# mrluin/TextualDegRemoval

Hardware: AMD Instinct MI355X
Metric: train images/sec (512x512, bs=4/GPU) (higher is better)
Workload: dtype f32 (3xbf16-split MFMA: 24-bit operand significands on the full fp32 exponent range, fp32 accumulate; unscaled gradients, no loss scale, no step-skip guard; tensors fp32 -- the MASA-encoder ResidualBlock activations / gradients as three bf16 planes whose sum IS the fp32 value, bit for bit)

## Files before the change

textualdegremoval_amd/csrc/tdr_wgrad_p16.hip:

```cpp
#include <stdlib.h>
#include <stdint.h>
#include "tdr_common.h"
#include "../../include/tdr.h"

typedef _Float16 wf16x8 __attribute__((ext_vector_type(8)));
typedef __bf16 wbf16x8 __attribute__((ext_vector_type(8)));
typedef short ws16x4 __attribute__((ext_vector_type(4)));
typedef short ws16x8 __attribute__((ext_vector_type(8)));

namespace {

struct WgP16Args {
    const uint4* in; const uint4* dout;
    int Cin, Cout, H, W, Hp, Wp;
    int strips, chunks, rc;
    float* part; float* dbpart;
    const void* grp_tab; int grp_pairs, grp_nsplit, grp_units, tiles_co, tiles_ci;
};

#define WGP_GLDS(gptr, lptr)                                                                          \
    __builtin_amdgcn_global_load_lds((__attribute__((address_space(1))) const void*)(gptr),          \
                                     (__attribute__((address_space(3))) void*)(lptr), 16, 0, 0)

__device__ __forceinline__ ws16x8 tr_frag(const char* p, int off0, int off1) {
    const ws16x4 a = __builtin_amdgcn_ds_read_tr16_b64_v4i16((__attribute__((address_space(3))) ws16x4*)(p + off0));
    const ws16x4 b = __builtin_amdgcn_ds_read_tr16_b64_v4i16((__attribute__((address_space(3))) ws16x4*)(p + off1));
    const ws16x8 v = {a[0], a[1], a[2], a[3], b[0], b[1], b[2], b[3]};
    return v;
}
template <int NS>
__device__ __forceinline__ f32x16 wg_mfma(ws16x8 x, ws16x8 y, f32x16 c) {
    if constexpr (NS == 3) return __builtin_amdgcn_mfma_f32_32x32x16_bf16(__builtin_bit_cast(wbf16x8, x), __builtin_bit_cast(wbf16x8, y), c, 0, 0, 0);
    else return __builtin_amdgcn_mfma_f32_32x32x16_f16(__builtin_bit_cast(wf16x8, x), __builtin_bit_cast(wf16x8, y), c, 0, 0, 0);
}

template <int WM, int WN, int WK, int NS = 2, bool GRP = false>
__global__ __launch_bounds__(256, 2) void wgrad3x3_p16_kernel(WgP16Args a) {
    static_assert(WM * WN * WK == 4, "4 waves");
    constexpr int RS = WK == 4 ? 2 : 1;
    static_assert(2 * RS % WK == 0, "k-steps of a step split evenly over the K waves");
    constexpr int BMo = 32 * WM, BNi = 32 * WN, NOo = BMo / 8, NOi = BNi / 8;
    constexpr int XS = 2 * RS + 2, DS = 2 * RS;
    constexpr int XR = ((NOi * NS * 34 + 63) / 64) * 64;
    constexpr int DR = NOo * NS * 32;
    constexpr int XP = XR / 64, DP = DR / 64;

    extern __shared__ __attribute__((aligned(1024))) uint4 smem4[];
    uint4* sX = smem4;
    uint4* sD = smem4 + XS * XR;

    const int tid = threadIdx.x, lane = tid & 63, wave = __builtin_amdgcn_readfirstlane(tid >> 6);
    const int wk = wave % WK, wn = (wave / WK) % WN, wm = wave / (WK * WN);
    int split = blockIdx.x, u0 = blockIdx.x, u1 = u0 + 1, tco = blockIdx.y, tci = blockIdx.z;
    float* dbout = a.dbpart;
    if constexpr (GRP) {
        const int T = a.tiles_co * a.tiles_ci;
        const int c8 = (int)blockIdx.x / (8 * T), r = (int)blockIdx.x - c8 * (8 * T);
        const int pair = c8 * 8 + (r & 7), tile = r >> 3;
        if (pair >= a.grp_pairs) return;
        const int prob = pair / a.grp_nsplit;
        split = pair - prob * a.grp_nsplit;
        tco = tile % a.tiles_co; tci = tile / a.tiles_co;
        u0 = (int)((long)split * a.grp_units / a.grp_nsplit);
        u1 = (int)((long)(split + 1) * a.grp_units / a.grp_nsplit);
        const TdrWg1GroupEntry e = static_cast<const TdrWg1GroupEntry*>(a.grp_tab)[prob];
        a.in = reinterpret_cast<const uint4*>(e.in); a.dout = reinterpret_cast<const uint4*>(e.dout);
        const bool direct = a.grp_nsplit == 1;
        a.part = direct ? e.g : e.part;
        dbout = direct ? e.db : e.dbpart;
    }
    const int co0 = tco * BMo, ci0 = tci * BNi;
    const long PS = (long)a.Hp * a.Wp;
    const int Gi = a.Cin >> 3, Go = a.Cout >> 3;
    const char* xbase = reinterpret_cast<const char*>(a.in);
    const char* dbase = reinterpret_cast<const char*>(a.dout);

    const int nn = lane & 15, g16 = lane >> 4;
    const int jpx = nn >> 2, q = nn & 3, chalf = g16 & 1, kk = g16 >> 1;
    const int oct = chalf * 2 + (q >> 1);
    const int a_lane = ((wm * 4 + oct) * NS * 32 + 8 * kk + jpx) * 16 + (q & 1) * 8;
    const int b_lane = ((wn * 4 + oct) * NS * 34 + 8 * kk + jpx) * 16 + (q & 1) * 8;

    f32x16 acc[9];
#pragma unroll
    for (int tp = 0; tp < 9; ++tp)
#pragma unroll
        for (int r = 0; r < 16; ++r) acc[tp][r] = 0.f;
    f32x16 accb;
#pragma unroll
    for (int r = 0; r < 16; ++r) accb[r] = 0.f;
    const bool want_db = dbout != nullptr && tci == 0 && wn == 0;
    ws16x8 ones;
#pragma unroll
    for (int e = 0; e < 8; ++e) ones[e] = NS == 3 ? (short)0x3f80 : (short)0x3c00;

    for (int u = u0; u < u1; ++u) {
        const int chunk = u % a.chunks; const int t = u / a.chunks;
        const int strip = t % a.strips;
        const int n = t / a.strips;
        const int y0 = chunk * a.rc, y1 = min(y0 + a.rc, a.H);
        const int x0 = strip * 32;

        constexpr int XPW = (XP + 3) / 4, DPW = (DP + 3) / 4;
        unsigned xoff[XPW], doff[DPW];
        const char* xb = xbase + (long)n * Gi * NS * PS * 16;
        const char* db = dbase + (long)n * Go * NS * PS * 16;
        bool dcol[DPW];
#pragma unroll
        for (int i = 0; i < XPW; ++i) {
            const int f = min((wave + 4 * i) * 64 + lane, NOi * NS * 34 - 1);
            const int op = f / 34, c = f - op * 34;
            const int oc = min((ci0 >> 3) + (op / NS), Gi - 1);
            xoff[i] = (unsigned)((((long)oc * NS + (op % NS)) * PS + min(x0 + c, a.Wp - 1)) * 16);
        }
#pragma unroll
        for (int i = 0; i < DPW; ++i) {
            const int f = (wave + 4 * i) * 64 + lane;
            const int op = f >> 5, c = f & 31;
            const int oc = min((co0 >> 3) + (op / NS), Go - 1);
            dcol[i] = x0 + c < a.W;
            doff[i] = (unsigned)((((long)oc * NS + (op % NS)) * PS) * 16);
        }
        auto glds = [&](const char* base, unsigned off, uint4* dst) {
            const unsigned l = (unsigned)(uintptr_t)(__attribute__((address_space(3))) char*)dst;
            unsigned keep;
            asm volatile("s_mov_b32 %0, m0\n\ts_mov_b32 m0, %2\n\ts_nop 0\n\tglobal_load_lds_dwordx4 %1, %3\n\ts_mov_b32 m0, %0"
                         : "=&s"(keep) : "v"(off), "s"(l), "s"(base) : "memory");
        };
        auto issue_x_row = [&](int prow) {
            uint4* dst = sX + (prow % XS) * XR;
            const long rowb = (long)min(prow, a.Hp - 1) * a.Wp * 16;
#pragma unroll
            for (int i = 0; i < XPW; ++i)
                if (wave + 4 * i < XP) glds(xb + rowb, xoff[i], dst + (wave + 4 * i) * 64);
        };
        auto issue_d_row = [&](int y) {
            uint4* dst = sD + (y % DS) * DR;
            const bool yok = y < a.H;
            const unsigned rowb = (unsigned)(((long)(y + 1) * a.Wp + x0 + 1) * 16);
#pragma unroll
            for (int i = 0; i < DPW; ++i)
                if (wave + 4 * i < DP) {
                    const int c = ((wave + 4 * i) * 64 + lane) & 31;
                    glds(db, doff[i] + ((yok && dcol[i]) ? rowb + c * 16 : 0u), dst + (wave + 4 * i) * 64);
                }
        };

        issue_x_row(y0); issue_x_row(y0 + 1);
#pragma unroll
        for (int r = 0; r < RS; ++r) { issue_x_row(y0 + 2 + r); issue_d_row(y0 + r); }
        asm volatile("s_waitcnt vmcnt(0) lgkmcnt(0)\n\ts_barrier" ::: "memory");

        for (int y = y0; y < y1; y += RS) {
#pragma unroll
            for (int r = 0; r < RS; ++r) { issue_x_row(y + RS + 2 + r); issue_d_row(y + RS + r); }
#pragma unroll
            for (int uu = 0; uu < 2 * RS / WK; ++uu) {
                const int ku = wk + uu * WK;
                const int yr = y + (ku >> 1), ks = ku & 1;
                if (yr < y1) {
                    const char* pd = reinterpret_cast<const char*>(sD + (yr % DS) * DR) + a_lane + ks * 256;
                    ws16x8 ap[NS];
#pragma unroll
                    for (int s = 0; s < NS; ++s) ap[s] = tr_frag(pd, s * 32 * 16, s * 32 * 16 + 64);
                    if (want_db) {
#pragma unroll
                        for (int s = NS - 1; s >= 0; --s) accb = wg_mfma<NS>(ap[s], ones, accb);
                    }
                    constexpr int NPR = NS == 3 ? 6 : 3;
                    constexpr int PA[6] = {NS == 3 ? 2 : 1, 0, NS == 3 ? 1 : 0, 1, 0, 0};
                    constexpr int PB[6] = {0, NS == 3 ? 2 : 1, NS == 3 ? 1 : 0, 0, 1, 0};
#pragma unroll
                    for (int ky = 0; ky < 3; ++ky) {
                        const char* px = reinterpret_cast<const char*>(sX + ((yr + ky) % XS) * XR) + b_lane + ks * 256;
                        ws16x8 bp[NS][3];
#pragma unroll
                        for (int s = 0; s < NS; ++s)
#pragma unroll
                            for (int kx = 0; kx < 3; ++kx) bp[s][kx] = tr_frag(px, s * 34 * 16 + kx * 16, s * 34 * 16 + kx * 16 + 64);
#pragma unroll
                        for (int pr = 0; pr < NPR; ++pr)
#pragma unroll
                            for (int kx = 0; kx < 3; ++kx) acc[ky * 3 + kx] = wg_mfma<NS>(ap[PA[pr]], bp[PB[pr]][kx], acc[ky * 3 + kx]);
                    }
                }
            }
            asm volatile("s_waitcnt vmcnt(0) lgkmcnt(0)\n\ts_barrier" ::: "memory");
        }
    }

    const int j = lane & 31, kg = lane >> 5;
    if constexpr (WK > 1) {
        float* red = reinterpret_cast<float*>(smem4);
#pragma unroll
        for (int w = 1; w < WK; ++w) {
            __syncthreads();
            if (wk == w) {
#pragma unroll
                for (int tp = 0; tp < 9; ++tp)
#pragma unroll
                    for (int r = 0; r < 16; ++r) red[(tp * 16 + r) * 64 + lane] = acc[tp][r];
#pragma unroll
                for (int r = 0; r < 16; ++r) red[(9 * 16 + r) * 64 + lane] = accb[r];
            }
            __syncthreads();
            if (wk == 0) {
#pragma unroll
                for (int tp = 0; tp < 9; ++tp)
#pragma unroll
                    for (int r = 0; r < 16; ++r) acc[tp][r] += red[(tp * 16 + r) * 64 + lane];
#pragma unroll
                for (int r = 0; r < 16; ++r) accb[r] += red[(9 * 16 + r) * 64 + lane];
            }
        }
        if (wk != 0) return;
    }
    float* part = a.part + (long)split * a.Cout * a.Cin * 9;
    const int ci = ci0 + wn * 32 + j;
#pragma unroll
    for (int r = 0; r < 16; ++r) {
        const int co = co0 + wm * 32 + (r & 3) + 8 * (r >> 2) + 4 * kg;
        if (co < a.Cout && ci < a.Cin) {
#pragma unroll
            for (int tp = 0; tp < 9; ++tp) part[((long)co * a.Cin + ci) * 9 + tp] = acc[tp][r];
        }
        if (want_db && j == 0 && co < a.Cout) dbout[(long)split * a.Cout + co] = accb[r];
    }
}

template <int KL>
__device__ __forceinline__ void wgp_reduce_block(const float* __restrict__ part, long elems, int nsplit, float* __restrict__ out, int nb_main,
                                                 const float* __restrict__ part2, long elems2, float* __restrict__ out2, int bx) {
    __shared__ float red[KL][64];
    const int lane = threadIdx.x & 63, kl = threadIdx.x >> 6;
    const bool second = bx >= nb_main;
    const float* pbase = second ? part2 : part;
    const long ne = second ? elems2 : elems;
    float* o = second ? out2 : out;
    const long e = (bx - (second ? nb_main : 0)) * 64L + lane;
    const float* p = pbase + (e < ne ? e : ne - 1);
    float s0 = 0.f;
    for (int k = kl; k < nsplit; k += 8 * KL) {
        float v[8];
#pragma unroll
        for (int u = 0; u < 8; ++u) v[u] = k + u * KL < nsplit ? p[(long)(k + u * KL) * ne] : 0.f;
        s0 += ((v[0] + v[1]) + (v[2] + v[3])) + ((v[4] + v[5]) + (v[6] + v[7]));
    }
    red[kl][lane] = s0;
    __syncthreads();
    if (kl == 0 && e < ne) {
        float t = 0.f;
#pragma unroll
        for (int q = 0; q < KL; ++q) t += red[q][lane];
        o[e] = t;
    }
}

template <int KL>
__global__ __launch_bounds__(64 * KL) void wgrad_p16_reduce_kernel(const float* __restrict__ part, long elems, int nsplit, float* __restrict__ out,
                                                                   int nb_main, const float* __restrict__ part2, long elems2, float* __restrict__ out2) {
    wgp_reduce_block<KL>(part, elems, nsplit, out, nb_main, part2, elems2, out2, (int)blockIdx.x);
}

template <int KL>
__global__ __launch_bounds__(64 * KL) void wgrad_p16_reduce_kernel_grp(const TdrWg1GroupEntry* __restrict__ tab, long elems, int nsplit, int Cout,
                                                                       int nb_main) {
    const TdrWg1GroupEntry e = tab[blockIdx.y];
    if ((int)blockIdx.x >= nb_main && (e.db == nullptr || e.dbpart == nullptr)) return;
    wgp_reduce_block<KL>(e.part, elems, nsplit, e.g, nb_main, e.dbpart, (long)Cout, e.db, (int)blockIdx.x);
}

struct WgP16Plan { int cfg, bm, bn, strips, chunks, rc, nsplit; };

long wgp_want_total() {
    static const long want_total = tdr_tune_env("TDR_WGP_WANT") ? atol(tdr_tune_env("TDR_WGP_WANT")) : 512;
    return want_total;
}

WgP16Plan wgp_plan_for(const TdrWgradP16Desc* d, long want) {
    WgP16Plan p;
    p.cfg = (d->Cin <= 32 && d->Cout <= 32) ? 1 : 0;
    p.bm = p.cfg == 1 ? 32 : 64; p.bn = p.bm;
    const int rs = p.cfg == 1 ? 2 : 1;
    p.strips = tdr_cdiv(d->W, 32);
    if (want < 1) want = 1;
    const long rows = (long)d->N * p.strips * d->H;
    long rc = (rows + want - 1) / want;
    if (rc < 8) rc = 8;
    rc = (rc + rs - 1) / rs * rs;
    if (rc > d->H) rc = (d->H + rs - 1) / rs * rs;
    p.rc = (int)rc;
    p.chunks = tdr_cdiv(d->H, p.rc);
    p.nsplit = d->N * p.strips * p.chunks;
    return p;
}

bool wgp_image_fits(const TdrWgradP16Desc* d) {
    const long c = d->Cin > d->Cout ? d->Cin : d->Cout;
    return c / 8 * 3 * (long)(d->H + 2) * (d->W + 2) * 16 < (1L << 32);
}

long wgp_out_tiles(const TdrWgradP16Desc* d) {
    const int t = (d->Cin <= 32 && d->Cout <= 32) ? 32 : 64;
    return (long)tdr_cdiv(d->Cout, t) * tdr_cdiv(d->Cin, t);
}

WgP16Plan wgp_plan(const TdrWgradP16Desc* d) { return wgp_plan_for(d, wgp_want_total() / wgp_out_tiles(d)); }

struct WgP16GroupPlan { WgP16Plan p; int units, nsplit; };

WgP16GroupPlan wgp_group_plan(const TdrWgradP16Desc* d, int nprob) {
    WgP16GroupPlan gp;
    long want = wgp_want_total() / ((long)nprob * wgp_out_tiles(d));
    if (want < 1) want = 1;
    gp.p = wgp_plan_for(d, want);
    gp.units = gp.p.nsplit;
    gp.nsplit = (int)(want < gp.units ? want : gp.units);
    return gp;
}

template <int WM, int WN, int WK, int NS, bool GRP = false>
int launch_wgp(const WgP16Args& a, const WgP16Plan& p, const TdrWgradP16Desc* d, hipStream_t st) {
    constexpr int RS = WK == 4 ? 2 : 1, NOo = 4 * WM, NOi = 4 * WN;
    constexpr int XR = ((NOi * NS * 34 + 63) / 64) * 64, DR = NOo * NS * 32;
    size_t lds = (size_t)((2 * RS + 2) * XR + 2 * RS * DR) * 16;
    if (WK > 1 && lds < 10 * 16 * 64 * 4) lds = 10 * 16 * 64 * 4;
    dim3 grid(p.nsplit, tdr_cdiv(d->Cout, 32 * WM), tdr_cdiv(d->Cin, 32 * WN));
    if (GRP) grid = dim3((unsigned)tdr_cdiv(a.grp_pairs, 8) * 8 * a.tiles_co * a.tiles_ci);
    auto kern = wgrad3x3_p16_kernel<WM, WN, WK, NS, GRP>;
    static bool attr_set = false;
    if (!attr_set) {
        (void)hipFuncSetAttribute(reinterpret_cast<const void*>(kern), hipFuncAttributeMaxDynamicSharedMemorySize, 160 * 1024);
        attr_set = true;
    }
    hipLaunchKernelGGL(kern, grid, dim3(256), lds, st, a);
    TDR_LAUNCH_CHECK(GRP ? "wgrad3x3_p16_kernel<grouped>" : "wgrad3x3_p16_kernel");
    return TDR_OK;
}

}

extern "C" int64_t tdr_wgrad3x3_p16_ws_floats(const TdrWgradP16Desc* d) {
    const WgP16Plan p = wgp_plan(d);
    return (int64_t)p.nsplit * d->Cout * d->Cin * 9 + (int64_t)p.nsplit * d->Cout;
}

extern "C" int tdr_wgrad3x3_p16(const TdrWgradP16Desc* d, void* stream) {
    TDR_REQUIRE(d && d->in16 && d->dout16 && d->g && d->ws, "tdr_wgrad3x3_p16: null pointer");
    TDR_REQUIRE(d->Cin % 16 == 0 && d->Cout % 16 == 0, "tdr_wgrad3x3_p16: channel counts must be multiples of 16 (%d, %d)", d->Cin, d->Cout);
    TDR_REQUIRE(wgp_image_fits(d), "tdr_wgrad3x3_p16: a plane image of more than 4 GiB");
    const WgP16Plan p = wgp_plan(d);
    const int64_t need = tdr_wgrad3x3_p16_ws_floats(d);
    TDR_REQUIRE(d->ws_floats >= need, "tdr_wgrad3x3_p16: workspace too small (%lld < %lld)", (long long)d->ws_floats, (long long)need);
    WgP16Args a;
    a.in = (const uint4*)d->in16; a.dout = (const uint4*)d->dout16;
    a.Cin = d->Cin; a.Cout = d->Cout; a.H = d->H; a.W = d->W; a.Hp = d->H + 2; a.Wp = d->W + 2;
    a.strips = p.strips; a.chunks = p.chunks; a.rc = p.rc;
    a.part = d->ws;
    a.grp_tab = nullptr; a.grp_pairs = a.grp_nsplit = a.grp_units = a.tiles_co = a.tiles_ci = 0;
    a.dbpart = d->db ? d->ws + (int64_t)p.nsplit * d->Cout * d->Cin * 9 : nullptr;
    hipStream_t st = (hipStream_t)stream;
    TDR_REQUIRE(d->fmt == 0 || d->fmt == 1 || d->fmt == 2, "tdr_wgrad3x3_p16: plane format %d (1: bf16 triple, 2: fp16 pair)", d->fmt);
    int rc;
    if (d->fmt == 1) rc = p.cfg == 1 ? launch_wgp<1, 1, 4, 3>(a, p, d, st) : launch_wgp<2, 2, 1, 3>(a, p, d, st);
    else rc = p.cfg == 1 ? launch_wgp<1, 1, 4, 2>(a, p, d, st) : launch_wgp<2, 2, 1, 2>(a, p, d, st);
    if (rc != TDR_OK) return rc;
    const long elems = (long)d->Cout * d->Cin * 9;
    const int nb_main = tdr_cdiv(elems, 64), nb2 = d->db ? tdr_cdiv(d->Cout, 64) : 0;
    if (p.nsplit <= 8)
        hipLaunchKernelGGL(wgrad_p16_reduce_kernel<1>, dim3(nb_main + nb2), dim3(64), 0, st, d->ws, elems, p.nsplit, d->g, nb_main, a.dbpart,
                           (long)d->Cout, d->db);
    else if (p.nsplit <= 64)
        hipLaunchKernelGGL(wgrad_p16_reduce_kernel<4>, dim3(nb_main + nb2), dim3(256), 0, st, d->ws, elems, p.nsplit, d->g, nb_main, a.dbpart,
                           (long)d->Cout, d->db);
    else
        hipLaunchKernelGGL(wgrad_p16_reduce_kernel<16>, dim3(nb_main + nb2), dim3(1024), 0, st, d->ws, elems, p.nsplit, d->g, nb_main, a.dbpart,
                           (long)d->Cout, d->db);
    TDR_LAUNCH_CHECK("wgrad_p16_reduce_kernel");
    return TDR_OK;
}

extern "C" int64_t tdr_wgrad3x3_p16_group_ws_floats(const TdrWgradP16Desc* d, int nprob) {
    if (!d || nprob < 1) return 0;
    const WgP16GroupPlan gp = wgp_group_plan(d, nprob);
    if (gp.nsplit == 1) return 0;
    return (int64_t)gp.nsplit * d->Cout * d->Cin * 9 + (int64_t)gp.nsplit * d->Cout;
}

extern "C" int tdr_wgrad3x3_p16_group_plan(const TdrWgradP16Desc* d, int nprob, int* nsplit, int* units, int* units_per_wg) {
    TDR_REQUIRE(d && nprob > 0, "tdr_wgrad3x3_p16_group_plan: null argument");
    const WgP16GroupPlan gp = wgp_group_plan(d, nprob);
    if (nsplit) *nsplit = gp.nsplit;
    if (units) *units = gp.units;
    if (units_per_wg) *units_per_wg = tdr_cdiv(gp.units, gp.nsplit);
    return TDR_OK;
}

extern "C" int tdr_wgrad3x3_p16_group(const TdrWgradP16Desc* d, int nprob, const void* table, void* stream) {
    TDR_REQUIRE(d && table && nprob > 0, "tdr_wgrad3x3_p16_group: null argument");
    TDR_REQUIRE(d->Cin % 16 == 0 && d->Cout % 16 == 0, "tdr_wgrad3x3_p16_group: channel counts must be multiples of 16 (%d, %d)", d->Cin, d->Cout);
    TDR_REQUIRE(d->fmt == 0 || d->fmt == 1 || d->fmt == 2, "tdr_wgrad3x3_p16_group: plane format %d (1: bf16 triple, 2: fp16 pair)", d->fmt);
    TDR_REQUIRE(wgp_image_fits(d), "tdr_wgrad3x3_p16_group: a plane image of more than 4 GiB");
    const WgP16GroupPlan gp = wgp_group_plan(d, nprob);
    const WgP16Plan& p = gp.p;
    WgP16Args a;
    a.in = nullptr; a.dout = nullptr; a.part = nullptr; a.dbpart = nullptr;
    a.Cin = d->Cin; a.Cout = d->Cout; a.H = d->H; a.W = d->W; a.Hp = d->H + 2; a.Wp = d->W + 2;
    a.strips = p.strips; a.chunks = p.chunks; a.rc = p.rc;
    a.grp_tab = table; a.grp_nsplit = gp.nsplit; a.grp_units = gp.units;
    a.tiles_co = tdr_cdiv(d->Cout, p.bm); a.tiles_ci = tdr_cdiv(d->Cin, p.bn);
    const long pairs = (long)nprob * gp.nsplit;
    TDR_REQUIRE(pairs * a.tiles_co * a.tiles_ci < (1L << 30), "tdr_wgrad3x3_p16_group: too many workgroups (%ld pairs)", pairs);
    a.grp_pairs = (int)pairs;
    hipStream_t st = (hipStream_t)stream;
    int rc;
    if (d->fmt == 1) rc = p.cfg == 1 ? launch_wgp<1, 1, 4, 3, true>(a, p, d, st) : launch_wgp<2, 2, 1, 3, true>(a, p, d, st);
    else rc = p.cfg == 1 ? launch_wgp<1, 1, 4, 2, true>(a, p, d, st) : launch_wgp<2, 2, 1, 2, true>(a, p, d, st);
    if (rc != TDR_OK || gp.nsplit == 1) return rc;
    const long elems = (long)d->Cout * d->Cin * 9;
    const int nb_main = tdr_cdiv(elems, 64), nb2 = tdr_cdiv(d->Cout, 64);
    const TdrWg1GroupEntry* tab = static_cast<const TdrWg1GroupEntry*>(table);
    if (gp.nsplit <= 8)
        hipLaunchKernelGGL(wgrad_p16_reduce_kernel_grp<1>, dim3(nb_main + nb2, nprob), dim3(64), 0, st, tab, elems, gp.nsplit, d->Cout, nb_main);
    else if (gp.nsplit <= 64)
        hipLaunchKernelGGL(wgrad_p16_reduce_kernel_grp<4>, dim3(nb_main + nb2, nprob), dim3(256), 0, st, tab, elems, gp.nsplit, d->Cout, nb_main);
    else
        hipLaunchKernelGGL(wgrad_p16_reduce_kernel_grp<16>, dim3(nb_main + nb2, nprob), dim3(1024), 0, st, tab, elems, gp.nsplit, d->Cout, nb_main);
    TDR_LAUNCH_CHECK("wgrad_p16_reduce_kernel_grp");
    return TDR_OK;
}
```

Before: 62.94.

## Pad and swizzle LDS layout, software-pipeline transposed reads against MFMAs in wgrad

Moves the wgrad LDS geometry into a shared layout header. For the 3-plane case the X-row pitch is padded from 34 to 36, and the dout rows get an XOR rotation by octet to reduce LDS bank conflicts on ds_read_tr. The inner tap loop is rewritten as a statically unrolled, double-buffered pipeline: B fragments for the next tap and A fragments for the next k-step load while the current tap's MFMAs issue. This is steered by sched_group_barrier and stepped s_setprio. It adds register pressure from the double buffers and a static_assert on the LDS budget, and it changes the fill and read addressing that both sides must agree on.

```diff
diff --git a/profiles/wgrad_p16_lds/compare_dumps.py b/profiles/wgrad_p16_lds/compare_dumps.py
--- /dev/null
+++ b/profiles/wgrad_p16_lds/compare_dumps.py
@@ -0,0 +1,17 @@
+import hashlib
+import os
+import sys
+
+import numpy as np
+
+a, b = sys.argv[1:3]
+bad = 0
+print(f'{a} vs {b}')
+for name in ('loss.npy', 'output.npy', 'params.npy'):
+    x, y = np.load(os.path.join(a, name)), np.load(os.path.join(b, name))
+    same = x.shape == y.shape and x.tobytes() == y.tobytes()
+    diff = '' if same else f' max|d|={np.abs(x.astype(np.float64) - y.astype(np.float64)).max():.3e}'
+    print(f'{name} {x.shape} {"IDENTICAL" if same else "DIFFERENT"}{diff} sha256 {hashlib.sha256(x.tobytes()).hexdigest()[:16]} / '
+          f'{hashlib.sha256(y.tobytes()).hexdigest()[:16]}')
+    bad += not same
+sys.exit(1 if bad else 0)
diff --git a/profiles/wgrad_p16_lds/hash_outputs.py b/profiles/wgrad_p16_lds/hash_outputs.py
--- /dev/null
+++ b/profiles/wgrad_p16_lds/hash_outputs.py
@@ -0,0 +1,29 @@
+import hashlib
+import os
+import sys
+
+ROOT = os.path.dirname(os.path.dirname(os.path.dirname(os.path.abspath(__file__))))
+sys.path.insert(0, ROOT)
+sys.path.insert(0, os.path.join(ROOT, 'tests'))
+import torch
+
+import test_hip_wgrad_p16_layout as T
+from textualdegremoval_amd import kernels as K
+
+
+def sha(t):
+    return hashlib.sha256(t.detach().cpu().contiguous().numpy().tobytes()).hexdigest()[:32]
+
+
+K.set_math('bx3')
+for fmt in T.FMTS:
+    for shape in T.SHAPES:
+        x16, d16 = T._planes(K, shape, fmt)
+        g, db = K.wgrad3x3_p16(x16, d16, want_db=True)
+        torch.cuda.synchronize()
+        print(f'single {fmt} {shape}: g {sha(g)} db {sha(db)}')
+    for shape, nprob, expect in T.GROUPS:
+        reqs = [T._planes(K, shape, fmt, i) for i in range(nprob)]
+        out = K.wgrad3x3_p16_group(reqs, seq=('hash', shape, fmt))
+        torch.cuda.synchronize()
+        print(f'group  {fmt} {shape} x{nprob} ({expect}): g {sha(torch.cat([g for g, _ in out]))} db {sha(torch.cat([db for _, db in out]))}')
diff --git a/profiles/wgrad_p16_lds/isa_report.py b/profiles/wgrad_p16_lds/isa_report.py
--- /dev/null
+++ b/profiles/wgrad_p16_lds/isa_report.py
@@ -0,0 +1,42 @@
+import re
+import sys
+
+s = open(sys.argv[1]).read()
+meta = {}
+for m in re.finditer(r'\.agpr_count:\s+(\d+).*?\.name:\s+(\S+).*?\.vgpr_count:\s+(\d+)\s+\.vgpr_spill_count:\s+(\d+)', s, re.S):
+    meta[m.group(2)] = (int(m.group(3)), int(m.group(1)), int(m.group(4)))
+for name in sorted(k for k in meta if 'wgrad3x3_p16_kernel' in k):
+    a = s.index(name + ':')
+    body = s[a:s.index('.Lfunc_end', a)].split('\n')
+    ops = []
+    for line in body:
+        t = line.strip()
+        if not t or t.startswith(';') or t.startswith('.'):
+            continue
+        op = t.split()[0]
+        if op.startswith('v_mfma'):
+            ops.append('M')
+        elif op.startswith('ds_read_b64_tr'):
+            ops.append('R')
+        elif op == 's_barrier':
+            ops.append('B')
+        elif op == 's_waitcnt':
+            m = re.search(r'lgkmcnt\((\d+)\)', t)
+            if m:
+                ops.append(int(m.group(1)))
+    cuts = [i for i, o in enumerate(ops) if o == 'B']
+    best = None
+    for i, j in zip(cuts, cuts[1:]):
+        seg = ops[i + 1:j]
+        if seg.count('M') and (best is None or seg.count('M') >= best.count('M')):
+            best = seg
+    nm = best.count('M')
+    first, last = best.index('M'), len(best) - 1 - best[::-1].index('M')
+    inner = best[first:last + 1]
+    waits = [o for o in inner if isinstance(o, int)]
+    per_tap = 6 if 'ELi3E' in name else 3
+    early0 = sum(1 for i, o in enumerate(inner) if o == 0 and inner[i:].count('M') > per_tap)
+    templ = re.search(r'kernelILi(\d)ELi(\d)ELi(\d)ELi(\d)ELb(\d)', name).groups()
+    v, ag, sp = meta[name]
+    print(f'wgrad3x3_p16_kernel<{", ".join(templ[:4])}, {"true" if templ[4] == "1" else "false"}>: vgpr {v} (agpr {ag}) spills {sp} | row loop: '
+          f'{nm} MFMA, {best.count("R")} tr-reads, lgkmcnt waits between first and last MFMA {waits}, lgkmcnt(0) ahead of more than the last tap: {early0}')
diff --git a/textualdegremoval_amd/csrc/tdr_wgrad_p16.hip b/textualdegremoval_amd/csrc/tdr_wgrad_p16.hip
--- a/textualdegremoval_amd/csrc/tdr_wgrad_p16.hip
+++ b/textualdegremoval_amd/csrc/tdr_wgrad_p16.hip
@@ -1,6 +1,8 @@
 #include <stdlib.h>
 #include <stdint.h>
+#include <type_traits>
 #include "tdr_common.h"
+#include "tdr_wgrad_p16_layout.h"
 #include "../../include/tdr.h"
 
 typedef _Float16 wf16x8 __attribute__((ext_vector_type(8)));
@@ -22,11 +24,18 @@
     __builtin_amdgcn_global_load_lds((__attribute__((address_space(1))) const void*)(gptr),          \
                                      (__attribute__((address_space(3))) void*)(lptr), 16, 0, 0)
 
-__device__ __forceinline__ ws16x8 tr_frag(const char* p, int off0, int off1) {
-    const ws16x4 a = __builtin_amdgcn_ds_read_tr16_b64_v4i16((__attribute__((address_space(3))) ws16x4*)(p + off0));
-    const ws16x4 b = __builtin_amdgcn_ds_read_tr16_b64_v4i16((__attribute__((address_space(3))) ws16x4*)(p + off1));
+__device__ __forceinline__ ws16x8 tr_frag(const char* p0, const char* p1) {
+    const ws16x4 a = __builtin_amdgcn_ds_read_tr16_b64_v4i16((__attribute__((address_space(3))) ws16x4*)p0);
+    const ws16x4 b = __builtin_amdgcn_ds_read_tr16_b64_v4i16((__attribute__((address_space(3))) ws16x4*)p1);
     const ws16x8 v = {a[0], a[1], a[2], a[3], b[0], b[1], b[2], b[3]};
     return v;
+}
+template <int I, int N, class F>
+__device__ __forceinline__ void wg_static_for(F&& f) {
+    if constexpr (I < N) {
+        f(std::integral_constant<int, I>{});
+        wg_static_for<I + 1, N>(f);
+    }
 }
 template <int NS>
 __device__ __forceinline__ f32x16 wg_mfma(ws16x8 x, ws16x8 y, f32x16 c) {
@@ -40,9 +49,11 @@
     constexpr int RS = WK == 4 ? 2 : 1;
     static_assert(2 * RS % WK == 0, "k-steps of a step split evenly over the K waves");
     constexpr int BMo = 32 * WM, BNi = 32 * WN, NOo = BMo / 8, NOi = BNi / 8;
-    constexpr int XS = 2 * RS + 2, DS = 2 * RS;
-    constexpr int XR = ((NOi * NS * 34 + 63) / 64) * 64;
-    constexpr int DR = NOo * NS * 32;
+    constexpr int XS = wgl::x_ring_rows(RS), DS = wgl::d_ring_rows(RS);
+    constexpr wgl::Layout L = wgl::layout(NS);
+    constexpr int XPI = L.xpitch;
+    constexpr int XR = wgl::x_row_slots(L, NOi);
+    constexpr int DR = wgl::d_row_slots(L, NOo);
     constexpr int XP = XR / 64, DP = DR / 64;
 
     extern __shared__ __attribute__((aligned(1024))) uint4 smem4[];
@@ -75,11 +86,8 @@
     const char* xbase = reinterpret_cast<const char*>(a.in);
     const char* dbase = reinterpret_cast<const char*>(a.dout);
 
-    const int nn = lane & 15, g16 = lane >> 4;
-    const int jpx = nn >> 2, q = nn & 3, chalf = g16 & 1, kk = g16 >> 1;
-    const int oct = chalf * 2 + (q >> 1);
-    const int a_lane = ((wm * 4 + oct) * NS * 32 + 8 * kk + jpx) * 16 + (q & 1) * 8;
-    const int b_lane = ((wn * 4 + oct) * NS * 34 + 8 * kk + jpx) * 16 + (q & 1) * 8;
+    const int a_lane0 = wgl::a_read_off(L, lane, wm, 0), a_lane1 = wgl::a_read_off(L, lane, wm, 1);
+    const int b_lane = wgl::b_read_off(L, lane, wn);
 
     f32x16 acc[9];
 #pragma unroll
@@ -105,21 +113,17 @@
         unsigned xoff[XPW], doff[DPW];
         const char* xb = xbase + (long)n * Gi * NS * PS * 16;
         const char* db = dbase + (long)n * Go * NS * PS * 16;
-        bool dcol[DPW];
+        int dcol[DPW];
 #pragma unroll
         for (int i = 0; i < XPW; ++i) {
-            const int f = min((wave + 4 * i) * 64 + lane, NOi * NS * 34 - 1);
-            const int op = f / 34, c = f - op * 34;
-            const int oc = min((ci0 >> 3) + (op / NS), Gi - 1);
-            xoff[i] = (unsigned)((((long)oc * NS + (op % NS)) * PS + min(x0 + c, a.Wp - 1)) * 16);
+            xoff[i] = wgl::x_src_off(L, NOi, (wave + 4 * i) * 64 + lane, ci0 >> 3, Gi, PS, x0, a.Wp);
         }
 #pragma unroll
         for (int i = 0; i < DPW; ++i) {
             const int f = (wave + 4 * i) * 64 + lane;
-            const int op = f >> 5, c = f & 31;
-            const int oc = min((co0 >> 3) + (op / NS), Go - 1);
-            dcol[i] = x0 + c < a.W;
-            doff[i] = (unsigned)((((long)oc * NS + (op % NS)) * PS) * 16);
+            const int c = wgl::d_fill(L, f).col;
+            dcol[i] = x0 + c < a.W ? c * 16 : -1;
+            doff[i] = wgl::d_src_plane_off(L, f, co0 >> 3, Go, PS);
         }
         auto glds = [&](const char* base, unsigned off, uint4* dst) {
             const unsigned l = (unsigned)(uintptr_t)(__attribute__((address_space(3))) char*)dst;
@@ -140,10 +144,7 @@
             const unsigned rowb = (unsigned)(((long)(y + 1) * a.Wp + x0 + 1) * 16);
 #pragma unroll
             for (int i = 0; i < DPW; ++i)
-                if (wave + 4 * i < DP) {
-                    const int c = ((wave + 4 * i) * 64 + lane) & 31;
-                    glds(db, doff[i] + ((yok && dcol[i]) ? rowb + c * 16 : 0u), dst + (wave + 4 * i) * 64);
-                }
+                if (wave + 4 * i < DP) glds(db, doff[i] + ((yok && dcol[i] >= 0) ? rowb + (unsigned)dcol[i] : 0u), dst + (wave + 4 * i) * 64);
         };
 
         issue_x_row(y0); issue_x_row(y0 + 1);
@@ -154,36 +155,55 @@
         for (int y = y0; y < y1; y += RS) {
 #pragma unroll
             for (int r = 0; r < RS; ++r) { issue_x_row(y + RS + 2 + r); issue_d_row(y + RS + r); }
-#pragma unroll
-            for (int uu = 0; uu < 2 * RS / WK; ++uu) {
-                const int ku = wk + uu * WK;
-                const int yr = y + (ku >> 1), ks = ku & 1;
-                if (yr < y1) {
-                    const char* pd = reinterpret_cast<const char*>(sD + (yr % DS) * DR) + a_lane + ks * 256;
-                    ws16x8 ap[NS];
-#pragma unroll
-                    for (int s = 0; s < NS; ++s) ap[s] = tr_frag(pd, s * 32 * 16, s * 32 * 16 + 64);
-                    if (want_db) {
-#pragma unroll
-                        for (int s = NS - 1; s >= 0; --s) accb = wg_mfma<NS>(ap[s], ones, accb);
+            constexpr int KSW = 2 * RS / WK, NT = 9 * KSW;
+            static_assert(KSW == 1 || RS == 1, "the k-steps of a wave lie in one row");
+            const int yr = y + (wk >> 1);
+            if (yr < y1) {
+                const char* pd = reinterpret_cast<const char*>(sD + (yr % DS) * DR);
+                const char* pd0 = pd + a_lane0, * pd1 = pd + a_lane1;
+                const char* px[3];
+#pragma unroll
+                for (int ky = 0; ky < 3; ++ky) px[ky] = reinterpret_cast<const char*>(sX + ((yr + ky) % XS) * XR) + b_lane;
+                auto ksb = [&](int uu) { return ((wk + uu * WK) & 1) * 256; };
+                auto ld_a = [&](ws16x8(&ap)[NS], int uu) {
+#pragma unroll
+                    for (int s = 0; s < NS; ++s) ap[s] = tr_frag(pd0 + ksb(uu) + s * 32 * 16, pd1 + ksb(uu) + s * 32 * 16);
+                };
+                auto ld_b = [&](ws16x8(&bp)[NS], int t) {
+                    const int uu = t / 9, ky = (t % 9) / 3, kx = t % 3;
+#pragma unroll
+                    for (int s = 0; s < NS; ++s) {
+                        const char* q = px[ky] + ksb(uu) + (s * XPI + kx) * 16;
+                        bp[s] = tr_frag(q, q + 64);
                     }
-                    constexpr int NPR = NS == 3 ? 6 : 3;
-                    constexpr int PA[6] = {NS == 3 ? 2 : 1, 0, NS == 3 ? 1 : 0, 1, 0, 0};
-                    constexpr int PB[6] = {0, NS == 3 ? 2 : 1, NS == 3 ? 1 : 0, 0, 1, 0};
-#pragma unroll
-                    for (int ky = 0; ky < 3; ++ky) {
-                        const char* px = reinterpret_cast<const char*>(sX + ((yr + ky) % XS) * XR) + b_lane + ks * 256;
-                        ws16x8 bp[NS][3];
-#pragma unroll
-                        for (int s = 0; s < NS; ++s)
-#pragma unroll
-                            for (int kx = 0; kx < 3; ++kx) bp[s][kx] = tr_frag(px, s * 34 * 16 + kx * 16, s * 34 * 16 + kx * 16 + 64);
-#pragma unroll
-                        for (int pr = 0; pr < NPR; ++pr)
-#pragma unroll
-                            for (int kx = 0; kx < 3; ++kx) acc[ky * 3 + kx] = wg_mfma<NS>(ap[PA[pr]], bp[PB[pr]][kx], acc[ky * 3 + kx]);
+                };
+                constexpr int NPR = NS == 3 ? 6 : 3;
+                constexpr int PA[6] = {NS == 3 ? 2 : 1, 0, NS == 3 ? 1 : 0, 1, 0, 0};
+                constexpr int PB[6] = {0, NS == 3 ? 2 : 1, NS == 3 ? 1 : 0, 0, 1, 0};
+                ws16x8 ap[2][NS], bp[2][NS];
+                ld_a(ap[0], 0);
+                ld_b(bp[0], 0);
+                __builtin_amdgcn_sched_barrier(0);
+                wg_static_for<0, NT>([&](auto tc) {
+                    constexpr int t = decltype(tc)::value, uu = t / 9, tp = t % 9;
+                    constexpr bool next_b = t + 1 < NT, next_a = tp == 7 && uu + 1 < KSW;
+                    constexpr int PQ = (NT + 3) / 4;
+                    if constexpr (t % PQ == 0) __builtin_amdgcn_s_setprio(t / PQ);
+                    if constexpr (next_b) ld_b(bp[(t + 1) & 1], t + 1);
+                    if constexpr (next_a) ld_a(ap[(uu + 1) & 1], uu + 1);
+#pragma unroll
+                    for (int pr = 0; pr < NPR; ++pr) acc[tp] = wg_mfma<NS>(ap[uu & 1][PA[pr]], bp[t & 1][PB[pr]], acc[tp]);
+                    if constexpr (next_b || next_a) __builtin_amdgcn_sched_group_barrier(0x100, (next_b ? 2 * NS : 0) + (next_a ? 2 * NS : 0), 0);
+                    __builtin_amdgcn_sched_group_barrier(0x008, NPR, 0);
+                    if constexpr (tp == 0) {
+                        if (want_db) {
+#pragma unroll
+                            for (int s = NS - 1; s >= 0; --s) accb = wg_mfma<NS>(ap[uu & 1][s], ones, accb);
+                        }
                     }
-                }
+                });
+                __builtin_amdgcn_sched_barrier(0);
+                __builtin_amdgcn_s_setprio(0);
             }
             asm volatile("s_waitcnt vmcnt(0) lgkmcnt(0)\n\ts_barrier" ::: "memory");
         }
@@ -322,8 +342,8 @@
 template <int WM, int WN, int WK, int NS, bool GRP = false>
 int launch_wgp(const WgP16Args& a, const WgP16Plan& p, const TdrWgradP16Desc* d, hipStream_t st) {
     constexpr int RS = WK == 4 ? 2 : 1, NOo = 4 * WM, NOi = 4 * WN;
-    constexpr int XR = ((NOi * NS * 34 + 63) / 64) * 64, DR = NOo * NS * 32;
-    size_t lds = (size_t)((2 * RS + 2) * XR + 2 * RS * DR) * 16;
+    size_t lds = (size_t)wgl::ring_bytes(wgl::layout(NS), NOo, NOi, RS);
+    static_assert(wgl::ring_bytes(wgl::layout(NS), NOo, NOi, RS) <= 80 * 1024, "two workgroups per CU");
     if (WK > 1 && lds < 10 * 16 * 64 * 4) lds = 10 * 16 * 64 * 4;
     dim3 grid(p.nsplit, tdr_cdiv(d->Cout, 32 * WM), tdr_cdiv(d->Cin, 32 * WN));
     if (GRP) grid = dim3((unsigned)tdr_cdiv(a.grp_pairs, 8) * 8 * a.tiles_co * a.tiles_ci);
diff --git a/textualdegremoval_amd/csrc/tdr_wgrad_p16_layout.h b/textualdegremoval_amd/csrc/tdr_wgrad_p16_layout.h
--- /dev/null
+++ b/textualdegremoval_amd/csrc/tdr_wgrad_p16_layout.h
@@ -0,0 +1,70 @@
+#ifndef TDR_WGRAD_P16_LAYOUT_H
+#define TDR_WGRAD_P16_LAYOUT_H
+
+#if defined(__HIPCC__) || defined(__CUDACC__)
+#define WGL_HD __host__ __device__ inline
+#else
+#define WGL_HD inline
+#endif
+
+namespace wgl {
+
+struct Layout {
+    int ns;
+    int xpitch;
+    bool drot;
+};
+
+WGL_HD constexpr Layout layout(int ns) { return Layout{ns, ns == 3 ? 36 : 34, true}; }
+
+WGL_HD constexpr int x_row_slots(Layout L, int noi) { return (noi * L.ns * L.xpitch + 63) / 64 * 64; }
+WGL_HD constexpr int d_row_slots(Layout L, int noo) { return noo * L.ns * 32; }
+WGL_HD constexpr int x_ring_rows(int rs) { return 2 * rs + 2; }
+WGL_HD constexpr int d_ring_rows(int rs) { return 2 * rs; }
+WGL_HD constexpr long ring_bytes(Layout L, int noo, int noi, int rs) {
+    return (long)(x_ring_rows(rs) * x_row_slots(L, noi) + d_ring_rows(rs) * d_row_slots(L, noo)) * 16;
+}
+
+WGL_HD constexpr int drot(Layout L, int octet) { return L.drot ? 4 * (octet & 3) : 0; }
+
+struct Elem { int octet, plane, col; };
+
+WGL_HD constexpr Elem x_fill(Layout L, int noi, int f) {
+    const int last = noi * L.ns * L.xpitch - 1;
+    const int g = f < last ? f : last;
+    const int op = g / L.xpitch;
+    return Elem{op / L.ns, op % L.ns, g - op * L.xpitch};
+}
+WGL_HD constexpr Elem d_fill(Layout L, int f) {
+    const int op = f >> 5, o = op / L.ns;
+    return Elem{o, op % L.ns, (f & 31) ^ drot(L, o)};
+}
+
+WGL_HD unsigned x_src_off(Layout L, int noi, int f, int oct0, int G, long PS, int x0, int Wp) {
+    const Elem e = x_fill(L, noi, f);
+    const int oc = oct0 + e.octet < G - 1 ? oct0 + e.octet : G - 1;
+    const int c = x0 + e.col < Wp - 1 ? x0 + e.col : Wp - 1;
+    return (unsigned)((((long)oc * L.ns + e.plane) * PS + c) * 16);
+}
+WGL_HD unsigned d_src_plane_off(Layout L, int f, int oct0, int G, long PS) {
+    const Elem e = d_fill(L, f);
+    const int oc = oct0 + e.octet < G - 1 ? oct0 + e.octet : G - 1;
+    return (unsigned)((((long)oc * L.ns + e.plane) * PS) * 16);
+}
+
+WGL_HD constexpr int lane_octet(int lane) { return ((lane >> 4) & 1) * 2 + ((lane & 3) >> 1); }
+WGL_HD constexpr int lane_pixel(int lane) { return 8 * (lane >> 5) + ((lane & 15) >> 2); }
+WGL_HD constexpr int lane_byte(int lane) { return (lane & 1) * 8; }
+
+WGL_HD constexpr int a_read_off(Layout L, int lane, int wm, int r) {
+    const int o = wm * 4 + lane_octet(lane);
+    const int px = lane_pixel(lane) + 4 * r;
+    return (o * L.ns * 32 + ((px & ~3) ^ drot(L, o)) + (px & 3)) * 16 + lane_byte(lane);
+}
+WGL_HD constexpr int b_read_off(Layout L, int lane, int wn) {
+    return ((wn * 4 + lane_octet(lane)) * L.ns * L.xpitch + lane_pixel(lane)) * 16 + lane_byte(lane);
+}
+
+}
+
+#endif
```

New measurement: 62.81. About the same (-0.2%).
